# polixir/emei

Measured on AMD Instinct MI355X. Metric: env-steps/s, higher is better.
Workload: dtype f64

## Files before the change

emei_amd/csrc/emei_device.h:

```cpp
#pragma once
#include <hip/hip_runtime.h>
#include <stdint.h>

#include "../../include/emei_hip.h"
#include "emei_math.h"

namespace emei {

constexpr int kBlock = 256;
constexpr int kWave = 64;

#if defined(EMEI_CLOCK_PROBE) && !defined(EMEI_NEWTON_STATS)
static __device__ unsigned long long g_debug_stats[32];
#endif
#ifdef EMEI_CLOCK_PROBE
#ifndef EMEI_CLOCK_BIN_TICKS
#define EMEI_CLOCK_BIN_TICKS 5000
#endif
struct ClockProbe {
    unsigned long long c0, r0;
    __device__ __forceinline__ void begin() { c0 = __builtin_readcyclecounter(), r0 = __builtin_amdgcn_s_memrealtime(); }
    __device__ __forceinline__ void end() const {
        const unsigned long long c1 = __builtin_readcyclecounter(), r1 = __builtin_amdgcn_s_memrealtime();
        if ((int)__lane_id() == __ffsll((unsigned long long)__ballot(1)) - 1) {
// ... 163 lines not shown
__device__ __forceinline__ void two_sum(double a, double b, double& s, double& e) {
    s = a + b;
    const double bb = s - a;
    e = (a - (s - bb)) + (b - bb);
}
__device__ __forceinline__ double trig_reduce_large(double x) {
    const double ax = __builtin_fabs(x);
    const double p2 = __builtin_amdgcn_trig_preop(ax, 0), p1 = __builtin_amdgcn_trig_preop(ax, 1),
                 p0 = __builtin_amdgcn_trig_preop(ax, 2);
    const double xs = ax >= 0x1.0p+945 ? __builtin_ldexp(ax, -128) : ax;
    double f2h = p2 * xs;
    const double f2l = __builtin_fma(p2, xs, -f2h);
    const double f1h = p1 * xs, f1l = __builtin_fma(p1, xs, -f1h);
    const double f0h = p0 * xs;
    const double q = __builtin_ldexp(f2h, -2);
    f2h = __builtin_ldexp(__builtin_amdgcn_fract(q), 2);
    double s1, e1, s2, e2;
    two_sum(f1h, f2l, s1, e1);
    two_sum(f2h, s1, s2, e2);
    const double low = ((f1l + f0h) + e1) + e2;
    const double k = __builtin_rint(s2);
    const double f = (s2 - k) + low;
    const double k4 = __builtin_fma(-4.0, __builtin_rint(k * 0.25), k);
    const double t = k4 + f;
    const double r = __builtin_fma(t, 6.123233995736766e-17, t * 1.5707963267948966);
    const double res = x < 0.0 ? -r : r;
    return __builtin_isfinite(x) ? res : __builtin_nan("");
}
__device__ __forceinline__ double trig_arg(double x) {
    const bool cold = !(__builtin_fabs(x) <= kFastTrigLimitF64);
    double r = x;
    if (__builtin_expect(__ballot(cold) != 0ull, 0)) {
        const double red = trig_reduce_large(x);
        r = cold ? red : x;
    }
    return r;
}

struct TrigCtx {
    const SinCosEntry* tab;
    double c3, c4;
    uint32_t lds_base;
    void* scratch = nullptr;
    int scratch_stride = kBlock;
    unsigned long long* cap_hits = nullptr;
};
__device__ __forceinline__ void report_cap_hit(const TrigCtx& t, bool hit) {
    if (__builtin_expect(__ballot(hit) != 0ull, 0)) {
        if (t.cap_hits) atomicAdd(t.cap_hits, hit ? 1ull : 0ull);
    }
}
__device__ __forceinline__ void trig_ctx_init(TrigCtx& t, const SinCosEntry* tab) {
    t.tab = tab;
    t.c3 = -1.0 / 6, t.c4 = 1.0 / 24;
    asm volatile("" : "+v"(t.c3), "+v"(t.c4));
    uint32_t base = __builtin_amdgcn_readfirstlane((uint32_t)(uintptr_t)(__attribute__((address_space(3))) const char*)tab);
    asm volatile("" : "+s"(base));
    t.lds_base = base;
}
__device__ __forceinline__ double fma_vsv(double a, double b_uniform, double c) {
    double d;
    asm("v_fma_f64 %0, %1, %2, %3" : "=v"(d) : "v"(a), "s"(b_uniform), "v"(c));
    return d;
}
__device__ __forceinline__ double fma_vvv(double a, double b, double c) {
    double d;
    asm("v_fma_f64 %0, %1, %2, %3" : "=v"(d) : "v"(a), "v"(b), "v"(c));
    return d;
}
__device__ __forceinline__ float fma_vvv(float a, float b, float c) { return __builtin_fmaf(a, b, c); }
__device__ __forceinline__ float fma_vsv(float a, float b, float c) { return __builtin_fmaf(a, b, c); }
__device__ __forceinline__ void sincos_fast_ctx(const TrigCtx& t, double x, double& s, double& c) {
    fast_sincos_tab(x, t.tab, s, c);
}
__device__ __forceinline__ void sincos_fast_ctx(const TrigCtx&, float x, float& s, float& c) { fast_sincosf(x, s, c); }
typedef double emei_d2 __attribute__((ext_vector_type(2)));
struct TrigPendingF64 {
    emei_d2 e;
    double sr, cr;
};
struct TrigPendingF32 {
    float s, c;
};
__device__ __forceinline__ TrigPendingF64 sincos_begin_ctx(const TrigCtx& t, double x_any) {
    const double inv_step = 40.74366543152521;
    const double H1 = 1.5707963267948966 / 64, H2 = 6.123233995736766e-17 / 64;
    auto begin = [&](double x) __attribute__((always_inline)) {
        TrigPendingF64 p;
        const double magic = 6755399441055744.0;
        const double shifted = __builtin_fma(x, inv_step, magic);
        const double n = shifted - magic;
        static_assert(kTrigTableSize == 256, "the index mask below");
        uint32_t addr;
        asm("v_and_b32 %0, 0xff, %1\n\tv_lshl_add_u32 %0, %0, 4, %2" : "=v"(addr) : "v"((uint32_t)__double2loint(shifted)), "s"(t.lds_base));
        asm volatile("ds_read_b128 %0, %1" : "=v"(p.e) : "v"(addr));
        double r = fma_vsv(n, -H1, x);
        r = __builtin_fma(-n, H2, r);
        const double z = r * r;
        p.sr = __builtin_fma(r * z, fma_vsv(z, 1.0 / 120, t.c3), r);
        p.cr = __builtin_fma(z, __builtin_fma(z, fma_vsv(z, -1.0 / 720, t.c4), -0.5), 1.0);
        return p;
    };
    TrigPendingF64 p = begin(x_any);
    const bool cold = !(__builtin_fabs(x_any) <= kFastTrigLimitF64);
    if (__builtin_expect(__ballot(cold) != 0ull, 0)) {
        asm volatile("s_waitcnt lgkmcnt(0)" : "+v"(p.e));
        const double red = trig_reduce_large(x_any);
        p = begin(cold ? red : x_any);
        asm volatile("s_waitcnt lgkmcnt(0)" : "+v"(p.e));
    }
    return p;
}
__device__ __forceinline__ void sincos_pin(const TrigPendingF64& p, double& a, double& b) {
    asm volatile("" : "+v"(a), "+v"(b) : "v"(p.e));
}
__device__ __forceinline__ void sincos_end_ctx(TrigPendingF64& p, double after0, double after1, double& s, double& c) {
    asm volatile("s_waitcnt lgkmcnt(0)" : "+v"(p.e) : "v"(after0), "v"(after1));
    s = __builtin_fma(p.e.x, p.cr, p.e.y * p.sr);
    c = __builtin_fma(p.e.y, p.cr, -(p.e.x * p.sr));
}
__device__ __forceinline__ TrigPendingF32 sincos_begin_ctx(const TrigCtx&, float x) {
    TrigPendingF32 p;
    fast_sincosf(x, p.s, p.c);
    return p;
}
__device__ __forceinline__ void sincos_pin(const TrigPendingF32&, float&, float&) {}
__device__ __forceinline__ void sincos_end_ctx(TrigPendingF32& p, float, float, float& s, float& c) { s = p.s, c = p.c; }

__device__ __forceinline__ void sincos_ctx(const TrigCtx& t, double x, double& s, double& c) {
    sincos_fast_ctx(t, trig_arg(x), s, c);
}
__device__ __forceinline__ void sincos_post_ctx(double, double&, double&) {}
__device__ __forceinline__ void sincos_post_ctx(float x, float& s, float& c) { sincos_repair_r(x, s, c); }
__device__ __forceinline__ void sincos_ctx(const TrigCtx& t, float x, float& s, float& c) {
    sincos_fast_ctx(t, x, s, c);
    sincos_repair_r(x, s, c);
}
template <int BLOCK = kBlock>
__device__ __forceinline__ void stage_trig_table(SinCosEntry* lds, const SinCosEntry* __restrict__ src, double rot_c = 1.0, double rot_s = 0.0) {
    static_assert(kTrigTableSize % BLOCK == 0, "every thread copies the same number of entries");
#pragma unroll
    for (int k = 0; k < kTrigTableSize / BLOCK; ++k) {
        SinCosEntry e = src[k * BLOCK + threadIdx.x];
        if (rot_s != 0.0) {
            const double sn = __builtin_fma(e.s, rot_c, e.c * rot_s), cs = __builtin_fma(e.c, rot_c, -(e.s * rot_s));
            e.s = sn, e.c = cs;
        } else if (rot_c != 1.0) {
            e.s *= rot_c, e.c *= rot_c;
        }
        lds[k * BLOCK + threadIdx.x] = e;
    }
    __syncthreads();
}

__device__ __forceinline__ double rcp_r(double d) { return refine_rcp(d, __builtin_amdgcn_rcp(d)); }
__device__ __forceinline__ float rcp_r(float d) { return 1.0f / d; }

__device__ __forceinline__ double rcp1_r(double d) {
    const double r0 = __builtin_amdgcn_rcp(d);
    return __builtin_fma(r0, __builtin_fma(-d, r0, 1.0), r0);
}
__device__ __forceinline__ float rcp1_r(float d) { return 1.0f / d; }
__device__ __forceinline__ double rsqrt_r(double x) {
    double r = __builtin_amdgcn_rsq(x);
    const double hx = 0.5 * x;
    r = __builtin_fma(r, __builtin_fma(-hx * r, r, 0.5), r);
    return __builtin_fma(r, __builtin_fma(-hx * r, r, 0.5), r);
}
__device__ __forceinline__ float rsqrt_r(float x) { return 1.0f / sqrtf(x); }
__device__ __forceinline__ double flip_sign(double v, uint32_t mask) {
    return __hiloint2double(__double2hiint(v) ^ (int)mask, __double2loint(v));
}
__device__ __forceinline__ float flip_sign(float v, uint32_t mask) { return __uint_as_float(__float_as_uint(v) ^ mask); }

__device__ __forceinline__ double abs_r(double x) { return __builtin_fabs(x); }
__device__ __forceinline__ float abs_r(float x) { return __builtin_fabsf(x); }
__device__ __forceinline__ double copysign_r(double mag, double sgn) { return __builtin_copysign(mag, sgn); }
__device__ __forceinline__ float copysign_r(float mag, float sgn) { return __builtin_copysignf(mag, sgn); }
__device__ __forceinline__ double fmax_r(double a, double b) { return __builtin_fmax(a, b); }
__device__ __forceinline__ float fmax_r(float a, float b) { return __builtin_fmaxf(a, b); }
__device__ __forceinline__ double fma_r(double a, double b, double c) { return __builtin_fma(a, b, c); }
__device__ __forceinline__ float fma_r(float a, float b, float c) { return __builtin_fmaf(a, b, c); }
__device__ __forceinline__ double div_r(double n, double d) { return n * rcp_r(d); }
__device__ __forceinline__ float div_r(float n, float d) { return n / d; }

template <typename T>
__device__ __forceinline__ T pymod_pos(T a, T p, T inv_p) {
    T k = floor(a * inv_p);
    T w = fma_r(-k, p, a);
    if (w < T(0)) w += p;
    else if (w >= p) w -= p;
    return w;
}

// ... 75 lines not shown
```

emei_amd/csrc/pendulum_envs.h:

```cpp
#pragma once
#include "constexpr_math.h"
#include "emei_device.h"

namespace emei {

struct PendParams {
    double dt;
    float dt32;
    float init_sigma[4];
    int32_t noise_shared;
    double M11, M22, mpr, mgr, gear, ctrl_lo, ctrl_hi, x_lo, x_hi;
    double sin_off, cos_off, phi_off;
    double invw, tc, dampratio, dmin, dmax, width;
    double limK, limB;
};

#ifndef EMEI_SPLIT_MAX_ROUNDS
#define EMEI_SPLIT_MAX_ROUNDS 3
#endif
template <int VARIANT, typename R>
struct CartPole {
    using real = R;
    static constexpr bool kDiscrete = true;
    static constexpr int kActDim = 1;
    struct Carry {
        R sn, cs;
        float xd32, td32;
        TrigCtx trig;
    };
    using Action = R;
    __host__ __device__ static constexpr double trig_rot_c() { return 1.0; }
    __host__ __device__ static constexpr double trig_rot_s() { return 0.0; }
    static constexpr bool kSpareInLds = false;
    static constexpr bool kSpareFlagInVgpr = false;
    static constexpr bool kRotatePriority = false;
    static constexpr bool kSplitLaunch = true;
    static constexpr unsigned kSplitMaxRounds = EMEI_SPLIT_MAX_ROUNDS;
    static constexpr bool kXcdContiguous = true;
    static constexpr bool kPeerWrite = true;
    static constexpr bool kTileBarrier = false;
    static constexpr bool kResetLikely = VARIANT == 1;
    static constexpr int kMinWavesPerEU = 1;
    struct Params {
        float dt32;
    };
    static Params make_params(const PendParams& p) { return Params{p.dt32}; }

    using RawAction = int;
    __device__ __forceinline__ static RawAction load_raw(const void* p, int dtype, int64_t idx) {
        return load_discrete_action(p, dtype, idx);
    }
    template <typename T>
    __device__ __forceinline__ static Action decode_t(T a) {
        return a == T(1) ? R(10.0 / 1.1) : R(-10.0 / 1.1);
    }
    __device__ __forceinline__ static Action decode(RawAction a) {
        return a == 1 ? R(10.0 / 1.1) : R(-10.0 / 1.1);
    }
    __device__ __forceinline__ static Action load_action(const void* p, int dtype, int64_t idx) {
        return decode(load_raw(p, dtype, idx));
    }

    __device__ __forceinline__ static void prime(const R s[4], Carry& c, const Params&) {
        sincos_ctx(c.trig, s[2], c.sn, c.cs);
        after_reset(s, c);
    }
    __device__ __forceinline__ static void after_reset(const R s[4], Carry& c) { c.xd32 = (float)s[1], c.td32 = (float)s[3]; }
    __device__ __forceinline__ static void save_extra(const Carry& c, float& e0, float& e1) { e0 = c.xd32, e1 = c.td32; }
    __device__ __forceinline__ static void load_extra(Carry& c, float e0, float e1) { c.xd32 = e0, c.td32 = e1; }

    __device__ __forceinline__ static void substep(R s[4], Carry& c, R force_over_m, const Params& p) {
        const R A = R(0.1 * 0.5 / 1.1);
        const R B = R(0.5 * 0.1 / 1.1);
        const R L43 = R(0.5 * 4.0 / 3.0);
        const R gravity = R(9.8);
        const R theta_dot = s[3];
        typedef float f32x2 __attribute__((ext_vector_type(2)));
        const f32x2 dpos = f32x2{c.xd32, c.td32} * p.dt32;
        s[0] += (R)dpos.x;
        s[2] += (R)dpos.y;
        R sn = c.sn, cs = c.cs;
        auto pending = sincos_begin_ctx(c.trig, s[2]);
        sincos_pin(pending, sn, cs);
        R temp = fma_vvv(A * (theta_dot * theta_dot), sn, force_over_m);
        R num = fma_r(gravity, sn, -(cs * temp));
        R den = fma_vsv(cs * cs, -B, L43);
        R theta_acc = div_r(num, den);
        R x_acc = fma_r(-(A * theta_acc), cs, temp);
        const f32x2 dvel = f32x2{(float)x_acc, (float)theta_acc} * p.dt32;
        s[1] += (R)dvel.x;
        s[3] += (R)dvel.y;
        c.xd32 = (float)s[1], c.td32 = (float)s[3];
        sincos_end_ctx(pending, x_acc, theta_acc, c.sn, c.cs);
        sincos_post_ctx(s[2], c.sn, c.cs);
    }

    __device__ __forceinline__ static void obs_of(const R s[4], R o[4]) {
        o[0] = s[0], o[1] = s[1], o[2] = s[2], o[3] = s[3];
    }

    __device__ __forceinline__ static R reward(const R o[4], const Carry& c, const Params&) {
        if (VARIANT == 0) return fma_r(c.cs, R(0.5), R(0.5));
        return R(1);
    }
    __device__ __forceinline__ static R reward_exact(const R o[4], const Carry& c, const Params& p) { return reward(o, c, p); }
    __device__ __forceinline__ static bool terminal(const R o[4], const Carry&, const Params&) {
        if (VARIANT == 0) {
            bool notdone = fabs(o[0]) < R(5);
            return !notdone;
        }
        const R theta_thr = R(12 * 2 * 3.141592653589793 / 360);
        bool notdone = (fabs(o[2]) < theta_thr) & (fabs(o[0]) < R(2.4));
        return !notdone;
    }

    __device__ __forceinline__ static void step(R s[4], Carry& c, Action force, const Params& p, int freq_rate,
                                                R o[4], R& rew, bool& term) {
        for (int k = 0; k < freq_rate; ++k) substep(s, c, force, p);
        obs_of(s, o);
        rew = reward(o, c, p);
        term = terminal(o, c, p);
    }

    __device__ __forceinline__ static void init(R s[4], uint64_t seed, uint64_t env, uint32_t episode,
                                                const Params&) {
        u32x4 r = philox4x32_10(seed, env, episode, 0);
        float f[4];
#pragma unroll
        for (int i = 0; i < 4; ++i) f[i] = __fmaf_rn(0.1f, u01(r.v[i]), -0.05f);
        if (VARIANT == 0) f[2] = __fadd_rn(f[2], 3.14159265358979323846f);
#pragma unroll
        for (int i = 0; i < 4; ++i) s[i] = (R)f[i];
    }
};

template <int VARIANT, typename R>
struct CartPoleRK4 : CartPole<VARIANT, R> {
    using Base = CartPole<VARIANT, R>;
    using real = R;
    using Carry = typename Base::Carry;
    using Params = typename Base::Params;
    using Action = R;

    __device__ __forceinline__ static void accel32(R theta_dot, R sn, R cs, R force_over_m, float& x_acc, float& theta_acc) {
        const R A = R(0.1 * 0.5 / 1.1), B = R(0.5 * 0.1 / 1.1), L43 = R(0.5 * 4.0 / 3.0), gravity = R(9.8);
        const R temp = fma_r(A * (theta_dot * theta_dot), sn, force_over_m);
        const R num = fma_r(gravity, sn, -(cs * temp));
        const R den = fma_r(cs * cs, -B, L43);
        const R ta = div_r(num, den);
        const R xa = fma_r(-(A * ta), cs, temp);
        x_acc = (float)xa, theta_acc = (float)ta;
    }

    __device__ __forceinline__ static void substep(R s[4], Carry& c, R force_over_m, const Params& p) {
        const float dt = p.dt32;
        float kxd[4], kxa[4], ktd[4], kta[4];
        kxd[0] = c.xd32, ktd[0] = c.td32;
        accel32(s[3], c.sn, c.cs, force_over_m, kxa[0], kta[0]);
#pragma unroll
        for (int st = 1; st < 4; ++st) {
            const float hxa = __fmul_rn(dt, kxa[st - 1]), htd = __fmul_rn(dt, ktd[st - 1]), hta = __fmul_rn(dt, kta[st - 1]);
            const float half = st < 3 ? 0.5f : 1.0f;
            const R xd = s[1] + (R)__fmul_rn(hxa, half), th = s[2] + (R)__fmul_rn(htd, half), td = s[3] + (R)__fmul_rn(hta, half);
            R sn, cs;
            sincos_ctx(c.trig, th, sn, cs);
            kxd[st] = (float)xd, ktd[st] = (float)td;
            accel32(td, sn, cs, force_over_m, kxa[st], kta[st]);
        }
        auto comb = [&](const float (&k)[4]) __attribute__((always_inline)) {
            const float a = __fadd_rn(k[0], __fmul_rn(2.0f, k[1]));
            const float b = __fadd_rn(a, __fmul_rn(2.0f, k[2]));
            return __fdiv_rn(__fmul_rn(__fadd_rn(b, k[3]), dt), 6.0f);
        };
        s[0] += (R)comb(kxd), s[1] += (R)comb(kxa), s[2] += (R)comb(ktd), s[3] += (R)comb(kta);
        c.xd32 = (float)s[1], c.td32 = (float)s[3];
        sincos_ctx(c.trig, s[2], c.sn, c.cs);
    }

    __device__ __forceinline__ static void step(R s[4], Carry& c, Action force, const Params& p, int freq_rate,
                                                R o[4], R& rew, bool& term) {
        for (int k = 0; k < freq_rate; ++k) substep(s, c, force, p);
        Base::obs_of(s, o);
        rew = Base::reward(o, c, p);
        term = Base::terminal(o, c, p);
    }
};

struct IpModel {
    double M11, M22, M11M22, mpr, inv_mpr, gravity, gear, ctrl_lo, ctrl_hi, x_lo, x_hi;
    double phi_off, sin_off, cos_off;
    double invw, dmin, dmax, inv_width;
    double mc, mp, Icom, r, phi0, solref_tc, width;
    double th_lo, th_hi, invw_hinge;
};
constexpr IpModel ip_make_model(bool swingup) {
    IpModel m{};
    const double rho = 1000.0, pi = ce::kPi;
    const auto capsule_mass = [&](double r, double half) { return rho * (pi * r * r * 2 * half + 4.0 / 3.0 * pi * r * r * r); };
    const auto capsule_inertia_perp = [&](double r, double half) {
        const double h = 2 * half, mcyl = rho * pi * r * r * h, msph = rho * 4.0 / 3.0 * pi * r * r * r;
        return mcyl * (3 * r * r + h * h) / 12 + msph * (2 * r * r / 5 + h * h / 4 + 3 * h * r / 8);
    };
    const double mc = capsule_mass(0.1, 0.1);
    const double fx = 0.001, fz = 0.6, len = ce::sqrt(fx * fx + fz * fz);
    const double mp = capsule_mass(0.049, len / 2), Icom = capsule_inertia_perp(0.049, len / 2), r = len / 2;
    const double phi0 = ce::atan_small(fx, fz);
    m.M11 = mc + mp, m.M22 = Icom + mp * r * r, m.M11M22 = m.M11 * m.M22;
    m.mpr = mp * r, m.inv_mpr = 1.0 / m.mpr, m.gravity = 9.81;
    m.gear = 100.0, m.ctrl_lo = -3.0, m.ctrl_hi = 3.0, m.x_lo = -2.0, m.x_hi = 2.0;
    m.phi_off = phi0 + (swingup ? pi : 0.0);
    m.sin_off = ce::sin(m.phi_off), m.cos_off = ce::cos(m.phi_off);
    const double M12 = m.mpr * ce::cos(phi0);
    m.invw = m.M22 / (m.M11 * m.M22 - M12 * M12);
    m.invw_hinge = m.M11 / (m.M11 * m.M22 - M12 * M12);
    m.th_lo = -pi / 2, m.th_hi = pi / 2;
    m.dmin = 0.9, m.dmax = 0.95, m.width = 0.001, m.inv_width = 1.0 / 0.001;
    m.mc = mc, m.mp = mp, m.Icom = Icom, m.r = r, m.phi0 = phi0, m.solref_tc = 0.02;
    return m;
}
__device__ constexpr IpModel kIpUpright = ip_make_model(false), kIpHanging = ip_make_model(true);

inline int ip_xml_constants(double* out) {
    constexpr IpModel m = ip_make_model(false);
    const double v[17] = {m.gravity, m.mc, m.mp, m.Icom, m.r, m.phi0, m.gear, m.ctrl_lo, m.ctrl_hi, m.x_lo, m.x_hi, m.solref_tc,
                          m.dmin, m.dmax, m.width, m.th_lo, m.th_hi};
// ... 5 lines not shown
__device__ __forceinline__ void ip_limit_rows(const IpModel& m, R x, R th, R v0, R v1, R M12, R idet, R limK, R limB, R& a0, R& a1) {
    R J[2], b[2], Rr[2];
    auto row = [&](int i, R qi, R vi, R lo, R hi, R invw, R ai) __attribute__((always_inline)) {
        const bool low = qi < lo, high = qi > hi, on = low | high;
        const R dist = low ? qi - lo : hi - qi;
        const R Ji = low ? R(1) : R(-1);
        const R xx = fabs(dist) * (R)m.inv_width;
        const R u1 = R(1) - xx;
        const R y = xx >= R(1) ? R(1) : (xx <= R(0.5) ? R(2) * xx * xx : fma_r(R(-2) * u1, u1, R(1)));
        const R imp = fma_r(y, (R)(m.dmax - m.dmin), (R)m.dmin);
        const R aref = fma_r(-limK * imp, dist, -limB * (Ji * vi));
        J[i] = on ? Ji : R(0);
        b[i] = on ? aref - Ji * ai : R(0);
        Rr[i] = on ? div_r(R(1) - imp, imp) * invw : R(1);
    };
    row(0, x, v0, (R)m.x_lo, (R)m.x_hi, (R)m.invw, a0);
    row(1, th, v1, (R)m.th_lo, (R)m.th_hi, (R)m.invw_hinge, a1);
    const bool has0 = J[0] != R(0), has1 = J[1] != R(0);
    const R A01 = J[0] * J[1] * (-M12 * idet);
    const R H00 = fma_r((R)m.M22, idet, Rr[0]), H11 = fma_r((R)m.M11, idet, Rr[1]);
    const R s0 = div_r(b[0], H00), s1 = div_r(b[1], H11);
    const R id2 = rcp_r(fma_r(H00, H11, -(A01 * A01)));
    const R t0 = fma_r(H11, b[0], -(A01 * b[1])) * id2, t1 = fma_r(H00, b[1], -(A01 * b[0])) * id2;
    const bool both = has0 & has1 & (t0 > R(0)) & (t1 > R(0));
    const bool only0 = !both & has0 & (s0 > R(0)) & !(has1 & (b[1] - A01 * s0 > R(0)));
    const bool only1 = !both & !only0 & has1 & (s1 > R(0)) & !(has0 & (b[0] - A01 * s1 > R(0)));
    const R f0 = both ? t0 : (only0 ? s0 : R(0)), f1 = both ? t1 : (only1 ? s1 : R(0));
    const R g0 = J[0] * f0, g1 = J[1] * f1;
    a0 = fma_r(fma_r((R)m.M22, g0, -(M12 * g1)), idet, a0);
    a1 = fma_r(fma_r((R)m.M11, g1, -(M12 * g0)), idet, a1);
}

template <typename R>
__device__ __forceinline__ void ip_limit_both(const IpModel& m, R x, R th, R v0, R v1, R M12, R idet, R limK, R limB, R& a0, R& a1) {
    auto row = [&](R qi, R vi, R lo, R hi, R invw, R Mdd, R ai, R& bi, R& Hii) __attribute__((always_inline)) {
        const bool low = qi < lo;
        const R dist = low ? qi - lo : hi - qi;
        const R xx = fabs(dist) * (R)m.inv_width;
        const R u1 = R(1) - xx;
        const R y = xx >= R(1) ? R(1) : (xx <= R(0.5) ? R(2) * xx * xx : fma_r(R(-2) * u1, u1, R(1)));
        const R imp = fma_r(y, (R)(m.dmax - m.dmin), (R)m.dmin);
        const R Jv = low ? vi : -vi, Ja = low ? ai : -ai;
        bi = fma_r(-limK * imp, dist, -limB * Jv) - Ja;
        Hii = fma_r(Mdd, idet, div_r(R(1) - imp, imp) * invw);
    };
    R b0, b1, H00, H11;
    row(x, v0, (R)m.x_lo, (R)m.x_hi, (R)m.invw, (R)m.M22, a0, b0, H00);
    row(th, v1, (R)m.th_lo, (R)m.th_hi, (R)m.invw_hinge, (R)m.M11, a1, b1, H11);
    const R mA = M12 * idet;
    const R A01 = ((x < (R)m.x_lo) == (th < (R)m.th_lo)) ? -mA : mA;
    const R id2 = rcp_r(fma_r(H00, H11, -(A01 * A01)));
    const R t0 = fma_r(H11, b0, -(A01 * b1)) * id2, t1 = fma_r(H00, b1, -(A01 * b0)) * id2;
    const bool both = (t0 > R(0)) & (t1 > R(0));
    const R s0 = div_r(b0, H00);
    const bool only0 = !both & (s0 > R(0)) & !(b1 - A01 * s0 > R(0));
    const R s1 = div_r(b1, H11);
    const bool only1 = !both & !only0 & (s1 > R(0)) & !(b0 - A01 * s1 > R(0));
    const R f0 = both ? t0 : (only0 ? s0 : R(0)), f1 = both ? t1 : (only1 ? s1 : R(0));
    const R g0 = x < (R)m.x_lo ? f0 : -f0, g1 = th < (R)m.th_lo ? f1 : -f1;
    a0 = fma_r(fma_r((R)m.M22, g0, -(M12 * g1)), idet, a0);
    a1 = fma_r(fma_r((R)m.M11, g1, -(M12 * g0)), idet, a1);
}

#ifndef EMEI_IP_XCD_CONTIGUOUS
#define EMEI_IP_XCD_CONTIGUOUS 0
#endif
#ifndef EMEI_IP_BAL_WAVES
#define EMEI_IP_BAL_WAVES 4
#endif
template <int VARIANT, typename R>
struct InvPend {
    using real = R;
    static constexpr bool kDiscrete = false;
    static constexpr int kActDim = 1;
    static constexpr bool kF64 = sizeof(R) == 8;
    static constexpr bool kSpareInLds = true;
    static constexpr bool kSpareFlagInVgpr = true;
    static constexpr bool kRotatePriority = true;
    static constexpr bool kSplitLaunch = false;
    static constexpr unsigned kSplitMaxRounds = 0;
    static constexpr bool kXcdContiguous = EMEI_IP_XCD_CONTIGUOUS != 0;
    static constexpr bool kPeerWrite = false;
    static constexpr bool kTileBarrier = false;
    static constexpr bool kResetLikely = true;
    static constexpr int kMinWavesPerEU = VARIANT >= 2 ? 4 : EMEI_IP_BAL_WAVES;
    __device__ static constexpr const IpModel& km() { return VARIANT >= 2 ? kIpHanging : kIpUpright; }
    __host__ __device__ static constexpr double trig_rot_c() { return kF64 ? ip_make_model(VARIANT >= 2).mpr * ip_make_model(VARIANT >= 2).cos_off : 1.0; }
    __host__ __device__ static constexpr double trig_rot_s() { return kF64 ? ip_make_model(VARIANT >= 2).mpr * ip_make_model(VARIANT >= 2).sin_off : 0.0; }
    __device__ __forceinline__ static R trig_angle(R theta) { return kF64 ? theta : theta + (R)km().phi_off; }
    struct Carry {
        R sn, cs;
        TrigCtx trig;
    };
    using Action = R;
    struct Params {
        double dt, limK, limB;
        float init_sigma[4];
        int32_t noise_shared;
    };
    static Params make_params(const PendParams& p) {
        Params q;
        q.dt = p.dt, q.limK = p.limK, q.limB = p.limB, q.noise_shared = p.noise_shared;
        for (int i = 0; i < 4; ++i) q.init_sigma[i] = p.init_sigma[i];
        return q;
    }

    using RawAction = float;
    __device__ __forceinline__ static RawAction load_raw(const void* p, int dtype, int64_t idx) {
        return (dtype == EMEI_ACT_F32) ? ((const float*)p)[idx] : (float)load_discrete_action(p, dtype, idx);
    }
    __device__ __forceinline__ static Action decode(RawAction a) {
        const float u = __builtin_amdgcn_fmed3f(a, (float)km().ctrl_lo, (float)km().ctrl_hi);
        return (R)km().gear * (R)u;
    }
    template <typename T>
    __device__ __forceinline__ static Action decode_t(T a) {
        return decode((float)a);
    }
    __device__ __forceinline__ static Action load_action(const void* p, int dtype, int64_t idx) {
        return decode(load_raw(p, dtype, idx));
    }

    __device__ __forceinline__ static void prime(const R s[4], Carry& c, const Params&) {
        sincos_ctx(c.trig, trig_angle(s[1]), c.sn, c.cs);
        if (!kF64) c.sn *= (R)km().mpr, c.cs *= (R)km().mpr;
    }
    __device__ __forceinline__ static void after_reset(const R[4], Carry&) {}
    __device__ __forceinline__ static void save_extra(const Carry&, float&, float&) {}
    __device__ __forceinline__ static void load_extra(Carry&, float, float) {}

    __device__ __forceinline__ static void substep(R s[4], Carry& c, R gu, const Params& p) {
        constexpr IpModel m = ip_make_model(VARIANT >= 2);
        const R dt = (R)p.dt;
        const R x_old = s[0], v_old = s[2], om_old = s[3];
        [[maybe_unused]] const R th_old = s[1];
        s[0] = fma_r(dt, v_old, x_old);
        s[1] = fma_r(dt, om_old, s[1]);
        R P = c.sn, Q = c.cs;
        auto pending = sincos_begin_ctx(c.trig, trig_angle(s[1]));
        sincos_pin(pending, P, Q);
        const R f1 = fma_r(P, om_old * om_old, gu);
        const R gP = (R)m.gravity * P;
        const R idet = rcp1_r(fma_r(-Q, Q, (R)m.M11M22));
        R a0 = fma_r((R)m.M22, f1, -(Q * gP)) * idet;
        R a1 = fma_r((R)m.M11, gP, -(Q * f1)) * idet;
        static_assert(m.x_lo == -m.x_hi, "symmetric slider range");
        const bool beyond = abs_r(x_old) > (R)m.x_hi;
        EMEI_STAT_WAVE(19);
        auto limit_row = [&](auto dof_c) __attribute__((always_inline)) {
            constexpr int DOF = decltype(dof_c)::value;
            constexpr double q_hi = DOF == 0 ? m.x_hi : m.th_hi, invw = DOF == 0 ? m.invw : m.invw_hinge, Mdd = DOF == 0 ? m.M22 : m.M11;
            const R qd = DOF == 0 ? x_old : th_old, vd = DOF == 0 ? v_old : om_old;
            R& ad = DOF == 0 ? a0 : a1;
            R& ao = DOF == 0 ? a1 : a0;
            if (DOF == 0) {
                EMEI_STAT_WAVE(20);
                EMEI_STAT_LANE(21);
            }
            const R nJ = copysign_r(R(1), qd);
            const R n1 = fma_r((R)p.limB, vd, ad);
            const R A = (R)Mdd * idet;
            constexpr double kRfull = (1.0 - m.dmax) / m.dmax * invw;
            const R Kfull = (R)p.limK * (R)m.dmax, Kfull_hi = Kfull * (R)q_hi;
            R kpos = fma_r(Kfull, abs_r(qd), -Kfull_hi);
            R den = A + (R)kRfull;
            const bool full = !(abs_r(qd) < (R)(q_hi + m.width));
// ... 93 lines not shown
```

emei_amd/csrc/pendulum_kernels.h:

```cpp
#pragma once
#include "pendulum_envs.h"
#include "launch.h"

namespace emei {

template <class Env>
struct RolloutArgs {
    typename Env::real* state;
    int32_t* steps;
    uint32_t* episode;
    unsigned long long* done_mask;
    const void* actions;
    const SinCosEntry* trig;
    float4* obs_out;
    float* reward_out;
    uint8_t* done_out;
    int64_t n;
    int32_t n_steps, freq_rate, action_dtype, max_episode_steps;
    uint32_t flags;
    uint64_t seed, env_offset;
    typename Env::Params p;
    double* obs_f64;
    uint32_t* host_flag;
    uint32_t flag_value;
// ... 19 lines not shown
    const uint32_t li = (uint32_t)i;

    R s[4];
#pragma unroll
    for (int k = 0; k < 4; ++k) s[k] = a.state[k * n + i];
    int32_t steps = a.steps[i];
    uint32_t episode = a.episode[i];
    typename Env::Carry c;
    trig_ctx_init(c.trig, trig_s);
    Env::prime(s, c, a.p);

    const bool auto_reset = (a.flags & EMEI_FLAG_AUTO_RESET) != 0;
    constexpr int kChunk = 8;
    const int last = a.n_steps - 1;
    ActT cur[kChunk], nxt[kChunk];
#pragma unroll
    for (int j = 0; j < kChunk; ++j) cur[j] = (actions + (int64_t)min(j, last) * n)[li];
    uint32_t done = 0;
    auto do_step = [&](int t, ActT raw) __attribute__((always_inline)) {
        R o[4], rew;
        bool term;
        Env::step(s, c, Env::decode_t(raw), a.p, a.freq_rate, o, rew, term);
        ++steps;
        bool trunc = (a.max_episode_steps > 0) & (steps >= a.max_episode_steps);
        done = (term ? EMEI_DONE_TERMINAL : 0u) | (trunc ? EMEI_DONE_TRUNCATED : 0u);

        const int64_t row = (int64_t)t * n;
        if (FULL || a.obs_out) (a.obs_out + row)[li] = make_float4((float)o[0], (float)o[1], (float)o[2], (float)o[3]);
        if (FULL || a.reward_out) (a.reward_out + row)[li] = (float)rew;
        if (FULL || a.done_out) (a.done_out + row)[li] = (uint8_t)done;

        if (auto_reset && __ballot(done != 0) != 0ull) {
            if (done != 0) {
                ++episode;
                steps = 0;
                Env::init(s, a.seed, a.env_offset + (uint64_t)i, episode, a.p);
                Env::prime(s, c, a.p);
            }
        }
    };
    int t0 = 0;
    for (; t0 + kChunk <= a.n_steps; t0 += kChunk) {
#pragma unroll
        for (int j = 0; j < kChunk; ++j) nxt[j] = (actions + (int64_t)min(t0 + kChunk + j, last) * n)[li];
#pragma unroll
        for (int j = 0; j < kChunk; ++j) do_step(t0 + j, cur[j]);
#pragma unroll
        for (int j = 0; j < kChunk; ++j) cur[j] = nxt[j];
    }
#pragma unroll
    for (int j = 0; j < kChunk; ++j) {
        if (t0 + j >= a.n_steps) break;
        do_step(t0 + j, cur[j]);
    }

#pragma unroll
    for (int k = 0; k < 4; ++k) a.state[k * n + i] = s[k];
    a.steps[i] = steps;
    a.episode[i] = episode;
    unsigned long long m = __ballot(done != 0);
    if ((threadIdx.x & (kWave - 1)) == 0) a.done_mask[i / kWave] = m;
    if (a.obs_f64) {
        R o[4];
        Env::obs_of(s, o);
        double2* dst = (double2*)(a.obs_f64 + 4 * i);
        dst[0] = make_double2((double)o[0], (double)o[1]);
        dst[1] = make_double2((double)o[2], (double)o[3]);
    }
    if (a.host_flag) {
        __threadfence_system();
        __hip_atomic_store(a.host_flag, a.flag_value, __ATOMIC_RELEASE, __HIP_MEMORY_SCOPE_SYSTEM);
    }
}

#ifndef EMEI_TILE_BARRIER
#define EMEI_TILE_BARRIER 1
#endif
#ifndef EMEI_PRIO_ROTATE
#define EMEI_PRIO_ROTATE 1
#endif
template <typename ActT>
constexpr int stage_steps() { return sizeof(ActT) == 1 ? 16 : 8; }

template <class Env, typename ActT, bool FREQ1, bool PEERS>
__device__ __forceinline__ void pend_rollout_staged(const RolloutArgs<Env>& a, const PeerObs& peers) {
    using R = typename Env::real;
    constexpr int kWavesPerBlock = kBlock / kWave;
    constexpr int kStage = stage_steps<ActT>();
    constexpr int kTileWaitKeep = kStage;
    constexpr int kActVec = kStage * sizeof(ActT) / 16;
    static_assert(kStage % 4 == 0 && kStage * kWave * sizeof(ActT) % 1024 == 0, "whole wave-loads, whole reward groups");
    __shared__ uint4 act_s[kWavesPerBlock][2][kStage * kWave * sizeof(ActT) / 16];
    __shared__ float rew_s[kWavesPerBlock][4][kWave];
    __shared__ uint8_t done_s[kWavesPerBlock][kStage][kWave];
    constexpr bool kLdsSpare = Env::kSpareInLds;
    __shared__ R spare_s[kLdsSpare ? kWavesPerBlock : 1][6][kLdsSpare ? kWave : 1];

    __shared__ SinCosEntry trig_s[kTrigTableSize];
    stage_trig_table(trig_s, a.trig, Env::trig_rot_c(), Env::trig_rot_s());
    const int lane = threadIdx.x & (kWave - 1), wv = threadIdx.x / kWave;
#if defined(EMEI_BLOCK_SWIZZLE)
    const int64_t i = (int64_t)((blockIdx.x + a.first_block) ^ (unsigned)EMEI_BLOCK_SWIZZLE) * kBlock + threadIdx.x;
#else
    const unsigned env_block = a.xcd_contiguous ? (blockIdx.x & 7u) * (gridDim.x >> 3) + (blockIdx.x >> 3) : blockIdx.x;
    const int64_t i = (int64_t)(env_block + a.first_block) * kBlock + threadIdx.x;
#endif
    if (i >= a.n) return;
#if defined(EMEI_XCD_ONLY)
    if (!(((unsigned)EMEI_XCD_ONLY >> (blockIdx.x & 7u)) & 1u)) return;
#endif
    EMEI_CLOCK_BEGIN();
    const int64_t n = a.n;
    const uint32_t li = (uint32_t)i, i0 = li - (uint32_t)lane;
    const ActT* __restrict__ actions = (const ActT*)a.actions;

    R s[4];
#pragma unroll
    for (int k = 0; k < 4; ++k) s[k] = a.state[k * n + i];
    int32_t steps = a.steps[i];
    uint32_t episode = a.episode[i];
    typename Env::Carry c;
    trig_ctx_init(c.trig, trig_s);
    Env::prime(s, c, a.p);
    const bool auto_reset = (a.flags & EMEI_FLAG_AUTO_RESET) != 0;
    const int last = a.n_steps - 1;
    uint32_t done = 0;

    constexpr int kLanesPerRow = kWave * sizeof(ActT) / 16;
    constexpr int kRowsPerVec = kWave / kLanesPerRow;
    const int rsub = lane / kLanesPerRow, cbyte = (lane % kLanesPerRow) * 16;
    const char* act_lane_base = (const char*)(actions + i0) + cbyte;
    const int64_t act_row_bytes = n * (int64_t)sizeof(ActT);
    const uint32_t act_lds0 = __builtin_amdgcn_readfirstlane(
        (uint32_t)(uintptr_t)(__attribute__((address_space(3))) char*)&act_s[wv][0][0]);
    constexpr uint32_t kTileBytes = kStage * kWave * sizeof(ActT);
#define EMEI_LOAD_TILE(T0, BUF)                                                                           \
    _Pragma("unroll") for (int k_ = 0; k_ < kActVec; ++k_) {                                             \
        const int row_ = min((T0) + k_ * kRowsPerVec + rsub, last);         \
        const char* src_ = act_lane_base + row_ * act_row_bytes;                                          \
        const uint32_t dst_ = act_lds0 + (uint32_t)(BUF) * kTileBytes + (uint32_t)k_ * 1024u;              \
        uint32_t keep_;                                                                                   \
        asm volatile("s_mov_b32 %0, m0\n\ts_mov_b32 m0, %2\n\ts_nop 0\n\tglobal_load_lds_dwordx4 %1, off\n\ts_mov_b32 m0, %0" \
                     : "=&s"(keep_) : "v"(src_), "s"(dst_) : "memory");                                    \
    }

    const int freq_rate = FREQ1 ? 1 : a.freq_rate;
    auto advance = [&](ActT raw, R (&o)[4], R& rew) __attribute__((always_inline)) {
        bool term;
        Env::step(s, c, Env::decode_t(raw), a.p, freq_rate, o, rew, term);
        ++steps;
        bool trunc = (a.max_episode_steps > 0) & (steps >= a.max_episode_steps);
        done = (term ? EMEI_DONE_TERMINAL : 0u) | (trunc ? EMEI_DONE_TRUNCATED : 0u);
    };
    R sp[4] = {R(0), R(0), R(0), R(0)}, sp_sn = R(0), sp_cs = R(0);
    float sp_e0 = 0.f, sp_e1 = 0.f;
    const unsigned long long reset_mask = auto_reset ? ~0ull : 0ull;
    constexpr bool kVFlag = Env::kSpareFlagInVgpr;
    unsigned long long spare_mask = 0ull;
    uint32_t spare_flag = 0u;
    auto maybe_reset = [&]() __attribute__((always_inline)) {
#if defined(EMEI_NO_RESET)
        return;
#endif
        EMEI_STAT_WAVE(16);
        const unsigned long long done_mask = __ballot(done != 0) & reset_mask;
        if (__builtin_expect(done_mask != 0ull, Env::kResetLikely ? 1 : 0)) {
            EMEI_STAT_WAVE(17);
            const bool refill = kVFlag ? (__ballot(done > spare_flag) & reset_mask) != 0ull : (done_mask & ~spare_mask) != 0ull;
            if (__builtin_expect(refill, 0)) {
                EMEI_STAT_WAVE(18);
                if (kVFlag ? spare_flag == 0u : __builtin_amdgcn_inverse_ballot_w64(~spare_mask)) {
                    typename Env::Carry sc;
                    sc.trig = c.trig;
                    Env::init(sp, a.seed, a.env_offset + (uint64_t)i, episode + 1u, a.p);
                    Env::prime(sp, sc, a.p);
                    if constexpr (kLdsSpare) {
                        spare_s[wv][0][lane] = sp[0], spare_s[wv][1][lane] = sp[1], spare_s[wv][2][lane] = sp[2];
                        spare_s[wv][3][lane] = sp[3], spare_s[wv][4][lane] = sc.sn, spare_s[wv][5][lane] = sc.cs;
                    } else {
                        sp_sn = sc.sn, sp_cs = sc.cs;
                        Env::save_extra(sc, sp_e0, sp_e1);
                    }
                }
                spare_mask = ~0ull, spare_flag = 3u;
            }
            if (__builtin_amdgcn_inverse_ballot_w64(done_mask)) {
                ++episode;
                steps = 0;
                if constexpr (kLdsSpare) {
                    s[0] = spare_s[wv][0][lane], s[1] = spare_s[wv][1][lane], s[2] = spare_s[wv][2][lane];
                    s[3] = spare_s[wv][3][lane], c.sn = spare_s[wv][4][lane], c.cs = spare_s[wv][5][lane];
                } else {
#pragma unroll
                    for (int k = 0; k < 4; ++k) s[k] = sp[k];
                    c.sn = sp_sn, c.cs = sp_cs;
                    Env::load_extra(c, sp_e0, sp_e1);
                }
                spare_flag = 0u;
            }
            spare_mask &= ~done_mask;
        }
    };
    const int64_t rew_lane_off = (int64_t)(lane >> 4) * n + i0 + ((lane & 15) << 2);
    const int64_t done_lane_off = (int64_t)(lane >> 2) * n + i0 + ((lane & 3) << 4);
#if defined(EMEI_EXP_FLUSH_ROW0)
#define EMEI_FLUSH_ROW(r) ((r) & 0)
#else
#define EMEI_FLUSH_ROW(r) (r)
#endif
    auto store_rew_rows = [&](int64_t row0, const float4& v) __attribute__((always_inline)) {
        store16_stream((float4*)(a.reward_out + EMEI_FLUSH_ROW(row0) * n + rew_lane_off), v);
    };
    auto store_done_rows = [&](int64_t row0, const uint4& v) __attribute__((always_inline)) {
        if (kStage == 16 || lane < 4 * kStage) store16_stream((uint4*)(a.done_out + EMEI_FLUSH_ROW(row0) * n + done_lane_off), v);
    };

    const uint32_t wave_slot = __builtin_amdgcn_s_getreg((4 - 1) << 11 | 0 << 6 | 4) & 3u;
    auto rotate_priority = [&](uint32_t tile) __attribute__((always_inline)) {
#if EMEI_PRIO_ROTATE
        if constexpr (Env::kRotatePriority) switch ((tile + wave_slot) & 3u) {
            case 0: __builtin_amdgcn_s_setprio(0); break;
            case 1: __builtin_amdgcn_s_setprio(1); break;
            case 2: __builtin_amdgcn_s_setprio(2); break;
            default: __builtin_amdgcn_s_setprio(3); break;
        }
#endif
    };
    auto store_obs_peers = [&](int t, const float4& v) __attribute__((always_inline)) {
        if constexpr (PEERS) {
            const int64_t at = (int64_t)t * peers.row_envs + peers.col + li;
            for (uint32_t p = 0; p < peers.count; ++p) peers.obs[p][at] = v;
        }
    };
    EMEI_LOAD_TILE(0, 0)
    asm volatile("s_waitcnt vmcnt(0)" ::: "memory");
    int t0 = 0, buf = 0;
    float4 rew_pend = make_float4(0.f, 0.f, 0.f, 0.f);
    uint4 done_pend = make_uint4(0u, 0u, 0u, 0u);
    for (; t0 + kStage <= a.n_steps; t0 += kStage, buf ^= 1) {
        EMEI_LOAD_TILE(t0 + kStage, buf ^ 1)
        rotate_priority((uint32_t)(t0 / kStage));
        const ActT* act_l = (const ActT*)&act_s[wv][buf][0];
        ActT act_cur = act_l[lane];
#ifndef EMEI_GROUP_UNROLL
#define EMEI_GROUP_UNROLL 2
#endif
#pragma unroll EMEI_GROUP_UNROLL
        for (int g = 0; g < kStage / 4; ++g) {
#pragma unroll
            for (int q = 0; q < 4; ++q) {
                const int j = 4 * g + q;
                const ActT act_now = act_cur;
                act_cur = act_l[min(j + 1, kStage - 1) * kWave + lane];
                R o[4], rew;
                advance(act_now, o, rew);
                const float4 obs4 = make_float4((float)o[0], (float)o[1], (float)o[2], (float)o[3]);
#if defined(EMEI_EXP_OBS_ROW0)
                (a.obs_out + (int64_t)((t0 + j) & 1) * n)[li] = obs4;
#else
                store16_stream(a.obs_out + (int64_t)(t0 + j) * n + li, obs4);
#endif
                store_obs_peers(t0 + j, obs4);
                if (q == 0) {
                    if (t0 + j > 0) store_rew_rows(t0 + j - 4, rew_pend);
                    if (g == 0 && t0 > 0) store_done_rows(t0 - kStage, done_pend);
                }
                rew_s[wv][q][lane] = (float)rew;
                done_s[wv][j][lane] = (uint8_t)done;
                if (q == 3) {
                    wave_lds_fence();
                    rew_pend = ((const float4*)&rew_s[wv][0][0])[lane];
                    if (g == kStage / 4 - 1) done_pend = ((const uint4*)&done_s[wv][0][0])[lane & (4 * kStage - 1)];
                    wave_lds_fence();
                }
                maybe_reset();
            }
        }
        static_assert(kTileWaitKeep == kStage && kTileWaitKeep < 64, "one unconditional obs store per staged step");
        asm volatile("s_waitcnt vmcnt(%0)" ::"i"(kTileWaitKeep) : "memory");
        if constexpr (EMEI_TILE_BARRIER != 0 && Env::kTileBarrier) __builtin_amdgcn_s_barrier();
    }
    if (t0 > 0) {
        store_rew_rows(t0 - 4, rew_pend);
        store_done_rows(t0 - kStage, done_pend);
    }
    for (int t = t0; t < a.n_steps; ++t) {
        R o[4], rew;
        advance((actions + (int64_t)t * n)[li], o, rew);
        const float4 obs4 = make_float4((float)o[0], (float)o[1], (float)o[2], (float)o[3]);
        (a.obs_out + (int64_t)t * n)[li] = obs4;
        store_obs_peers(t, obs4);
        (a.reward_out + (int64_t)t * n)[li] = (float)rew;
        (a.done_out + (int64_t)t * n)[li] = (uint8_t)done;
        maybe_reset();
    }

#pragma unroll
    for (int k = 0; k < 4; ++k) a.state[k * n + i] = s[k];
    a.steps[i] = steps;
    a.episode[i] = episode;
    unsigned long long m = __ballot(done != 0);
    if (lane == 0) a.done_mask[i / kWave] = m;
    EMEI_CLOCK_END();
#undef EMEI_LOAD_TILE
}

template <class Env, typename ActT, bool FREQ1>
__global__ void __launch_bounds__(kBlock) __attribute__((amdgpu_waves_per_eu(Env::kMinWavesPerEU)))
    pend_rollout_staged_kernel(const RolloutArgs<Env> a) {
    pend_rollout_staged<Env, ActT, FREQ1, false>(a, PeerObs{});
}

template <class Env, typename ActT, bool FREQ1>
__global__ void __launch_bounds__(kBlock) __attribute__((amdgpu_waves_per_eu(Env::kMinWavesPerEU)))
    pend_rollout_staged_peers_kernel(const RolloutArgs<Env> a, const PeerObs peers) {
    pend_rollout_staged<Env, ActT, FREQ1, true>(a, peers);
}

template <class Env>
__global__ void __launch_bounds__(kBlock)
    pend_reset_kernel(typename Env::real* state, int32_t* steps, uint32_t* episode, int64_t n, uint64_t seed,
                      uint64_t env_offset, typename Env::Params p) {
    using R = typename Env::real;
    const int64_t i = (int64_t)blockIdx.x * kBlock + threadIdx.x;
    if (i >= n) return;
    R s[4];
    Env::init(s, seed, env_offset + (uint64_t)i, 0u, p);
#pragma unroll
    for (int k = 0; k < 4; ++k) state[k * n + i] = s[k];
    steps[i] = 0;
    episode[i] = 0;
}

template <class Env>
__global__ void __launch_bounds__(kBlock)
    pend_init_obs_kernel(const int64_t* env_index, const uint32_t* episode, float4* obs, int64_t count, uint64_t seed,
                         uint64_t env_offset, typename Env::Params p) {
    using R = typename Env::real;
    const int64_t k = (int64_t)blockIdx.x * kBlock + threadIdx.x;
    if (k >= count) return;
    R s[4], o[4];
    Env::init(s, seed, env_offset + (uint64_t)env_index[k], episode[k], p);
    Env::obs_of(s, o);
    obs[k] = make_float4((float)o[0], (float)o[1], (float)o[2], (float)o[3]);
}

template <class Env>
__global__ void __launch_bounds__(kBlock)
    pend_get_obs_kernel(const typename Env::real* state, double* obs, int64_t n) {
    using R = typename Env::real;
    const int64_t i = (int64_t)blockIdx.x * kBlock + threadIdx.x;
    if (i >= n) return;
    R s[4], o[4];
#pragma unroll
    for (int k = 0; k < 4; ++k) s[k] = state[k * n + i];
    Env::obs_of(s, o);
    double2* dst = (double2*)(obs + 4 * i);
    dst[0] = make_double2((double)o[0], (double)o[1]);
// ... 299 lines not shown
```

Before: 273.9 billion.

## Defer large-angle trig repair and merge it with the reset exit in CartPole f64

```diff
diff --git a/emei_amd/csrc/emei_device.h b/emei_amd/csrc/emei_device.h
--- a/emei_amd/csrc/emei_device.h
+++ b/emei_amd/csrc/emei_device.h
@@ -269,10 +269,10 @@
 struct TrigPendingF32 {
     float s, c;
 };
-__device__ __forceinline__ TrigPendingF64 sincos_begin_ctx(const TrigCtx& t, double x_any) {
+__device__ __forceinline__ TrigPendingF64 sincos_table_begin(const TrigCtx& t, double x) {
     const double inv_step = 40.74366543152521;
     const double H1 = 1.5707963267948966 / 64, H2 = 6.123233995736766e-17 / 64;
-    auto begin = [&](double x) __attribute__((always_inline)) {
+    {
         TrigPendingF64 p;
         const double magic = 6755399441055744.0;
         const double shifted = __builtin_fma(x, inv_step, magic);
@@ -287,7 +287,10 @@
         p.sr = __builtin_fma(r * z, fma_vsv(z, 1.0 / 120, t.c3), r);
         p.cr = __builtin_fma(z, __builtin_fma(z, fma_vsv(z, -1.0 / 720, t.c4), -0.5), 1.0);
         return p;
-    };
+    }
+}
+__device__ __forceinline__ TrigPendingF64 sincos_begin_ctx(const TrigCtx& t, double x_any) {
+    auto begin = [&](double x) __attribute__((always_inline)) { return sincos_table_begin(t, x); };
     TrigPendingF64 p = begin(x_any);
     const bool cold = !(__builtin_fabs(x_any) <= kFastTrigLimitF64);
     if (__builtin_expect(__ballot(cold) != 0ull, 0)) {
@@ -297,6 +300,17 @@
         asm volatile("s_waitcnt lgkmcnt(0)" : "+v"(p.e));
     }
     return p;
+}
+__device__ __forceinline__ TrigPendingF64 sincos_begin_deferred(const TrigCtx& t, double x_any, bool& cold) {
+    cold = !(__builtin_fabs(x_any) <= kFastTrigLimitF64);
+    return sincos_table_begin(t, x_any);
+}
+__device__ __forceinline__ void sincos_repair_deferred(const TrigCtx& t, double x_any, bool cold, double& s, double& c) {
+    const double red = trig_reduce_large(x_any);
+    TrigPendingF64 p = sincos_table_begin(t, cold ? red : x_any);
+    asm volatile("s_waitcnt lgkmcnt(0)" : "+v"(p.e));
+    const double s2 = __builtin_fma(p.e.x, p.cr, p.e.y * p.sr), c2 = __builtin_fma(p.e.y, p.cr, -(p.e.x * p.sr));
+    s = cold ? s2 : s, c = cold ? c2 : c;
 }
 __device__ __forceinline__ void sincos_pin(const TrigPendingF64& p, double& a, double& b) {
     asm volatile("" : "+v"(a), "+v"(b) : "v"(p.e));
diff --git a/emei_amd/csrc/pendulum_envs.h b/emei_amd/csrc/pendulum_envs.h
--- a/emei_amd/csrc/pendulum_envs.h
+++ b/emei_amd/csrc/pendulum_envs.h
@@ -41,6 +41,7 @@
     static constexpr bool kTileBarrier = false;
     static constexpr bool kResetLikely = VARIANT == 1;
     static constexpr int kMinWavesPerEU = 1;
+    static constexpr bool kColdExit = sizeof(R) == 8;
     struct Params {
         float dt32;
     };
@@ -70,6 +71,11 @@
     __device__ __forceinline__ static void load_extra(Carry& c, float e0, float e1) { c.xd32 = e0, c.td32 = e1; }
 
     __device__ __forceinline__ static void substep(R s[4], Carry& c, R force_over_m, const Params& p) {
+        bool cold;
+        substep_t<false>(s, c, force_over_m, p, cold);
+    }
+    template <bool DEFER>
+    __device__ __forceinline__ static void substep_t(R s[4], Carry& c, R force_over_m, const Params& p, bool& cold) {
         const R A = R(0.1 * 0.5 / 1.1);
         const R B = R(0.5 * 0.1 / 1.1);
         const R L43 = R(0.5 * 4.0 / 3.0);
@@ -80,7 +86,10 @@
         s[0] += (R)dpos.x;
         s[2] += (R)dpos.y;
         R sn = c.sn, cs = c.cs;
-        auto pending = sincos_begin_ctx(c.trig, s[2]);
+        auto pending = [&]() __attribute__((always_inline)) {
+            if constexpr (DEFER) return sincos_begin_deferred(c.trig, s[2], cold);
+            else return sincos_begin_ctx(c.trig, s[2]);
+        }();
         sincos_pin(pending, sn, cs);
         R temp = fma_vvv(A * (theta_dot * theta_dot), sn, force_over_m);
         R num = fma_r(gravity, sn, -(cs * temp));
@@ -122,6 +131,20 @@
         term = terminal(o, c, p);
     }
 
+    __device__ __forceinline__ static void step_deferred(R s[4], Carry& c, Action force, const Params& p, R o[4], R& rew, bool& term,
+                                                         bool& cold) {
+        substep_t<true>(s, c, force, p, cold);
+        obs_of(s, o);
+        rew = reward(o, c, p);
+        term = terminal(o, c, p);
+    }
+    __device__ __forceinline__ static void repair_deferred(const R s[4], Carry& c, bool cold, const Params& p, R& rew) {
+        sincos_repair_deferred(c.trig, s[2], cold, c.sn, c.cs);
+        R o[4];
+        obs_of(s, o);
+        rew = reward(o, c, p);
+    }
+
     __device__ __forceinline__ static void init(R s[4], uint64_t seed, uint64_t env, uint32_t episode,
                                                 const Params&) {
         u32x4 r = philox4x32_10(seed, env, episode, 0);
@@ -141,6 +164,7 @@
     using Carry = typename Base::Carry;
     using Params = typename Base::Params;
     using Action = R;
+    static constexpr bool kColdExit = false;
 
     __device__ __forceinline__ static void accel32(R theta_dot, R sn, R cs, R force_over_m, float& x_acc, float& theta_acc) {
         const R A = R(0.1 * 0.5 / 1.1), B = R(0.5 * 0.1 / 1.1), L43 = R(0.5 * 4.0 / 3.0), gravity = R(9.8);
@@ -312,6 +336,7 @@
     static constexpr bool kXcdContiguous = EMEI_IP_XCD_CONTIGUOUS != 0;
     static constexpr bool kPeerWrite = false;
     static constexpr bool kTileBarrier = false;
+    static constexpr bool kColdExit = false;
     static constexpr bool kResetLikely = true;
     static constexpr int kMinWavesPerEU = VARIANT >= 2 ? 4 : EMEI_IP_BAL_WAVES;
     __device__ static constexpr const IpModel& km() { return VARIANT >= 2 ? kIpHanging : kIpUpright; }
diff --git a/emei_amd/csrc/pendulum_kernels.h b/emei_amd/csrc/pendulum_kernels.h
--- a/emei_amd/csrc/pendulum_kernels.h
+++ b/emei_amd/csrc/pendulum_kernels.h
@@ -125,6 +125,24 @@
 template <typename ActT>
 constexpr int stage_steps() { return sizeof(ActT) == 1 ? 16 : 8; }
 
+#ifndef EMEI_DONE_FROM_MASKS
+#define EMEI_DONE_FROM_MASKS 1
+#endif
+__device__ __forceinline__ uint32_t done_code_masks(int32_t steps, int32_t max_m1, unsigned long long term_mask, uint32_t two,
+                                                    unsigned long long& done_mask) {
+    static_assert(EMEI_DONE_TERMINAL == 1u && EMEI_DONE_TRUNCATED == 2u, "the done code as a sum");
+    uint32_t d;
+    asm("v_cmp_lt_i32_e32 vcc, %3, %2\n\t"
+        "v_cndmask_b32_e32 %0, 0, %5, vcc\n\t"
+        "s_or_b64 %1, vcc, %4\n\t"
+        "s_mov_b64 vcc, %4\n\t"
+        "v_addc_co_u32_e32 %0, vcc, 0, %0, vcc"
+        : "=&v"(d), "=&s"(done_mask)
+        : "v"(steps), "s"(max_m1), "s"(term_mask), "v"(two)
+        : "vcc", "scc");
+    return d;
+}
+
 template <class Env, typename ActT, bool FREQ1, bool PEERS>
 __device__ __forceinline__ void pend_rollout_staged(const RolloutArgs<Env>& a, const PeerObs& peers) {
     using R = typename Env::real;
@@ -244,6 +262,64 @@
             spare_mask &= ~done_mask;
         }
     };
+    constexpr bool kColdExit = Env::kColdExit;
+    const int32_t max_m1 = kColdExit ? (a.max_episode_steps > 0 ? a.max_episode_steps - 1 : INT32_MAX) : 0;
+    [[maybe_unused]] uint32_t v_two = EMEI_DONE_TRUNCATED;
+    if constexpr (kColdExit) asm volatile("" : "+v"(v_two));
+    auto advance_deferred = [&](ActT raw, R (&o)[4], R& rew, bool& cold, unsigned long long& done_any) __attribute__((always_inline)) {
+        if constexpr (kColdExit) {
+            bool term;
+            if constexpr (FREQ1) {
+                Env::step_deferred(s, c, Env::decode_t(raw), a.p, o, rew, term, cold);
+            } else {
+                Env::step(s, c, Env::decode_t(raw), a.p, freq_rate, o, rew, term);
+                cold = false;
+            }
+            ++steps;
+#if EMEI_DONE_FROM_MASKS
+            done = done_code_masks(steps, max_m1, __ballot(term), v_two, done_any);
+#else
+            const bool trunc = steps > max_m1;
+            done = (trunc ? EMEI_DONE_TRUNCATED : 0u) | (term ? EMEI_DONE_TERMINAL : 0u);
+            done_any = __ballot(term) | __ballot(trunc);
+#endif
+        }
+    };
+    auto cold_exit = [&](unsigned long long cold_mask, unsigned long long done_mask, bool cold, float* slot) __attribute__((always_inline)) {
+        if constexpr (kColdExit) {
+            asm volatile("s_waitcnt lgkmcnt(0)" ::: "memory");
+            if (FREQ1 && __builtin_expect(cold_mask != 0ull, 0)) {
+                R rew;
+                Env::repair_deferred(s, c, cold, a.p, rew);
+                *slot = (float)rew;
+            }
+            if (done_mask != 0ull) {
+                EMEI_STAT_WAVE(17);
+                if (__builtin_expect((done_mask & ~spare_mask) != 0ull, 0)) {
+                    EMEI_STAT_WAVE(18);
+                    if (__builtin_amdgcn_inverse_ballot_w64(~spare_mask)) {
+                        typename Env::Carry sc;
+                        sc.trig = c.trig;
+                        Env::init(sp, a.seed, a.env_offset + (uint64_t)i, episode + 1u, a.p);
+                        Env::prime(sp, sc, a.p);
+                        sp_sn = sc.sn, sp_cs = sc.cs;
+                        Env::save_extra(sc, sp_e0, sp_e1);
+                    }
+                    spare_mask = ~0ull;
+                }
+                if (__builtin_amdgcn_inverse_ballot_w64(done_mask)) {
+                    ++episode;
+                    steps = 0;
+#pragma unroll
+                    for (int k = 0; k < 4; ++k) s[k] = sp[k];
+                    c.sn = sp_sn, c.cs = sp_cs;
+                    Env::load_extra(c, sp_e0, sp_e1);
+                }
+                spare_mask &= ~done_mask;
+            }
+        }
+    };
+    static_assert(!kColdExit || (!kLdsSpare && !kVFlag), "the cold exit keeps its spares in registers and their flags in a scalar mask");
     const int64_t rew_lane_off = (int64_t)(lane >> 4) * n + i0 + ((lane & 15) << 2);
     const int64_t done_lane_off = (int64_t)(lane >> 2) * n + i0 + ((lane & 3) << 4);
 #if defined(EMEI_EXP_FLUSH_ROW0)
@@ -296,7 +372,10 @@
                 const ActT act_now = act_cur;
                 act_cur = act_l[min(j + 1, kStage - 1) * kWave + lane];
                 R o[4], rew;
-                advance(act_now, o, rew);
+                [[maybe_unused]] bool cold = false;
+                [[maybe_unused]] unsigned long long done_any = 0ull;
+                if constexpr (kColdExit) advance_deferred(act_now, o, rew, cold, done_any);
+                else advance(act_now, o, rew);
                 const float4 obs4 = make_float4((float)o[0], (float)o[1], (float)o[2], (float)o[3]);
 #if defined(EMEI_EXP_OBS_ROW0)
                 (a.obs_out + (int64_t)((t0 + j) & 1) * n)[li] = obs4;
@@ -310,13 +389,24 @@
                 }
                 rew_s[wv][q][lane] = (float)rew;
                 done_s[wv][j][lane] = (uint8_t)done;
+                if constexpr (kColdExit) {
+                    EMEI_STAT_WAVE(16);
+#if defined(EMEI_NO_RESET)
+                    const unsigned long long done_mask = 0ull;
+#else
+                    const unsigned long long done_mask = done_any & reset_mask;
+#endif
+                    const unsigned long long cold_mask = FREQ1 ? __ballot(cold) : 0ull;
+                    if (__builtin_expect((done_mask | cold_mask) != 0ull, Env::kResetLikely ? 1 : 0))
+                        cold_exit(cold_mask, done_mask, cold, &rew_s[wv][q][lane]);
+                }
                 if (q == 3) {
                     wave_lds_fence();
                     rew_pend = ((const float4*)&rew_s[wv][0][0])[lane];
                     if (g == kStage / 4 - 1) done_pend = ((const uint4*)&done_s[wv][0][0])[lane & (4 * kStage - 1)];
                     wave_lds_fence();
                 }
-                maybe_reset();
+                if constexpr (!kColdExit) maybe_reset();
             }
         }
         static_assert(kTileWaitKeep == kStage && kTileWaitKeep < 64, "one unconditional obs store per staged step");
```

Measured after the change: 271.7 billion. No clear change (-0.8%).
